# twice154/ofa-for-super-resolution

Hardware: AMD Instinct MI355X
Metric: sr_training_images_per_sec_4x_64to256 (higher is better)
Workload: dtype bf16; 1 GPU; OFA-SR S4 supernet 4x progressive shrinking (elastic kernel {3,5,7}, e=6, d=4, pd=2), LR 64x64 -> HR 256x256, fwd+bwd+Adam, train-mode BN; kernel_transform_mode=1, compat_reference_indexing=True, parallelism=dp1, per_gpu_batch=16, global_batch=16, grad_allreduce_bytes=0, launch=eager

## Files before the change

### ofa-for-super-resolution_amd/csrc/dwconv.hip

```cpp
#include "ofasr_common.h"

#include <type_traits>

namespace ofasr {

constexpr int DW_WAVES = 4;

template <int D>
__device__ __forceinline__ float lane_shift(float v, int lane) {
    if (D == 0) return v;
    const int src = lane + D;
    const float t = __shfl(v, src & 63, 64);
    return (src >= 0 && src < 64) ? t : 0.f;
}

template <int K>
struct Strips {
    static constexpr int PAD = K / 2;
    static __host__ __device__ int count(int W) { return W <= 64 ? 1 : (W + (64 - 2 * PAD) - 1) / (64 - 2 * PAD); }
    static __device__ int col0(int W, int s) { return W <= 64 ? 0 : s * (64 - 2 * PAD) - PAD; }
    static __device__ bool core(int W, int lane) { return W <= 64 ? true : (lane >= PAD && lane < 64 - PAD); }
};

template <typename T, int K, bool FLIP>
__global__ void __launch_bounds__(64 * DW_WAVES) dw_strip_kernel(const T* __restrict__ x, const float* __restrict__ f,
                                                                 T* __restrict__ y, int C, int H, int W,
                                                                 int nstrips, int nchunks, int rows_per_chunk,
                                                                 long long units) {
    constexpr int PAD = K / 2;
    const int lane = lane_id();
    const int wave = __builtin_amdgcn_readfirstlane((int)(threadIdx.x >> 6));
    const long long unit = (long long)blockIdx.x * DW_WAVES + wave;
    if (unit >= units) return;
    const int chunk = (int)(unit % nchunks);
    const long long u2 = unit / nchunks;
    const int strip = (int)(u2 % nstrips);
    const long long plane = u2 / nstrips;
    const int c = (int)(plane % C);

    float taps[K * K];
#pragma unroll
    for (int e = 0; e < K * K; ++e) taps[e] = f[(long long)c * K * K + (FLIP ? (K * K - 1 - e) : e)];

    const int col = Strips<K>::col0(W, strip) + lane;
    const bool in_col = col >= 0 && col < W;
    const bool out_col = in_col && Strips<K>::core(W, lane);
    const int h0 = chunk * rows_per_chunk;
    const int h1 = min(H, h0 + rows_per_chunk);
    const T* xp = x + plane * (long long)H * W + col;
    T* yp = y + plane * (long long)H * W + col;

    float acc[K];
#pragma unroll
    for (int i = 0; i < K; ++i) acc[i] = 0.f;

    const int hstart = h0 - PAD;
    const int niter = (h1 - h0) + 2 * PAD;
    auto load_row = [&](int t) -> float {
        const int hin = hstart + t;
        return (t < niter && hin >= 0 && hin < H && in_col) ? to_float(xp[(long long)hin * W]) : 0.f;
    };
    float xin[K], xnext[K];
#pragma unroll
    for (int u = 0; u < K; ++u) xin[u] = load_row(u);
    for (int base = 0; base < niter; base += K) {
#pragma unroll
        for (int u = 0; u < K; ++u) xnext[u] = load_row(base + K + u);
#pragma unroll
        for (int u = 0; u < K; ++u) {
            const int t = base + u;
            const int hin = hstart + t;
            const float v = xin[u];
            float s[K];
#pragma unroll
            for (int j = 0; j < K; ++j) {
                switch (j - PAD) {
                    case -3: s[j] = lane_shift<-3>(v, lane); break;
                    case -2: s[j] = lane_shift<-2>(v, lane); break;
                    case -1: s[j] = lane_shift<-1>(v, lane); break;
                    case 0: s[j] = v; break;
                    case 1: s[j] = lane_shift<1>(v, lane); break;
                    case 2: s[j] = lane_shift<2>(v, lane); break;
                    default: s[j] = lane_shift<3>(v, lane); break;
                }
            }
#pragma unroll
            for (int i = 0; i < K; ++i) {
                float a = acc[(u - i + K) % K];
#pragma unroll
                for (int j = 0; j < K; ++j) a = fmaf(taps[i * K + j], s[j], a);
                acc[(u - i + K) % K] = a;
            }
            const int hout = hin - PAD;
            if (t < niter && hout >= h0 && hout < h1 && out_col)
                yp[(long long)hout * W] = from_float<T>(acc[(u + 1) % K]);
            acc[(u + 1) % K] = 0.f;
        }
#pragma unroll
        for (int u = 0; u < K; ++u) xin[u] = xnext[u];
    }
}

template <typename T, int K>
__global__ void __launch_bounds__(64 * DW_WAVES) dw_wgrad_kernel(const T* __restrict__ dy, const T* __restrict__ x,
                                                                 float* __restrict__ part_out, int N, int C, int H,
                                                                 int W, int nstrips, int nparts, long long units) {
    constexpr int PAD = K / 2;
    const int lane = lane_id();
    const int wave = __builtin_amdgcn_readfirstlane((int)(threadIdx.x >> 6));
    const long long unit = (long long)blockIdx.x * DW_WAVES + wave;
    if (unit >= units) return;
    const int part = (int)(unit % nparts);
    const int c = (int)(unit / nparts);

    float acc[K * K];
#pragma unroll
    for (int e = 0; e < K * K; ++e) acc[e] = 0.f;

    for (int n = part; n < N; n += nparts) {
        const long long plane = (long long)n * C + c;
        for (int strip = 0; strip < nstrips; ++strip) {
            const int col = Strips<K>::col0(W, strip) + lane;
            const bool in_col = col >= 0 && col < W;
            const bool own = in_col && Strips<K>::core(W, lane);
            const T* dp = dy + plane * (long long)H * W + col;
            const T* xp = x + plane * (long long)H * W + col;
            float xr[K];
#pragma unroll
            for (int m = 0; m < K - 1; ++m) {
                const int r = m - PAD;
                xr[m] = (own && r >= 0 && r < H) ? to_float(xp[(long long)r * W]) : 0.f;
            }
            xr[K - 1] = 0.f;
            auto load_x = [&](int h) -> float {
                const int rnew = h + PAD;
                return (own && h < H && rnew < H) ? to_float(xp[(long long)rnew * W]) : 0.f;
            };
            auto load_g = [&](int h) -> float { return (h < H && in_col) ? to_float(dp[(long long)h * W]) : 0.f; };
            float xb[K], gb[K], xn_[K], gn_[K];
#pragma unroll
            for (int u = 0; u < K; ++u) {
                xb[u] = load_x(u);
                gb[u] = load_g(u);
            }
            for (int base = 0; base < H; base += K) {
#pragma unroll
                for (int u = 0; u < K; ++u) {
                    xn_[u] = load_x(base + K + u);
                    gn_[u] = load_g(base + K + u);
                }
#pragma unroll
                for (int u = 0; u < K; ++u) {
                    xr[(u + K - 1) % K] = xb[u];
                    const float g = gb[u];
                    float gs[K];
#pragma unroll
                    for (int j = 0; j < K; ++j) {
                        switch (PAD - j) {
                            case -3: gs[j] = lane_shift<-3>(g, lane); break;
                            case -2: gs[j] = lane_shift<-2>(g, lane); break;
                            case -1: gs[j] = lane_shift<-1>(g, lane); break;
                            case 0: gs[j] = g; break;
                            case 1: gs[j] = lane_shift<1>(g, lane); break;
                            case 2: gs[j] = lane_shift<2>(g, lane); break;
                            default: gs[j] = lane_shift<3>(g, lane); break;
                        }
                    }
#pragma unroll
                    for (int i = 0; i < K; ++i) {
                        const float xv = xr[(u + i) % K];
#pragma unroll
                        for (int j = 0; j < K; ++j) acc[i * K + j] = fmaf(gs[j], xv, acc[i * K + j]);
                    }
                }
#pragma unroll
                for (int u = 0; u < K; ++u) {
                    xb[u] = xn_[u];
                    gb[u] = gn_[u];
                }
            }
        }
    }
    float* out = part_out + ((long long)part * C + c) * (K * K);
#pragma unroll
    for (int e = 0; e < K * K; ++e) {
        const float s = wave_sum(acc[e]);
        if (lane == 0) out[e] = s;
    }
}

template <typename T, int PXL> struct PxIO;
template <> struct PxIO<float, 4> {
    typedef uint4 raw_t;
    static __device__ __forceinline__ raw_t zero() { return make_uint4(0, 0, 0, 0); }
    static __device__ __forceinline__ void unpack(const raw_t& v, float* o) {
        o[0] = __uint_as_float(v.x); o[1] = __uint_as_float(v.y); o[2] = __uint_as_float(v.z); o[3] = __uint_as_float(v.w);
    }
    static __device__ __forceinline__ raw_t pack(const float* i) {
        return make_uint4(__float_as_uint(i[0]), __float_as_uint(i[1]), __float_as_uint(i[2]), __float_as_uint(i[3]));
    }
};
template <typename T> struct PxIO<T, 8> {
    typedef uint4 raw_t;
    static __device__ __forceinline__ raw_t zero() { return make_uint4(0, 0, 0, 0); }
    static __device__ __forceinline__ void unpack(const raw_t& v, float* o) {
        const uint32_t w[4] = {v.x, v.y, v.z, v.w};
#pragma unroll
        for (int i = 0; i < 4; ++i) {
            T lo, hi;
            lo.v = (uint16_t)(w[i] & 0xffffu);
            hi.v = (uint16_t)(w[i] >> 16);
            o[2 * i] = to_float(lo);
            o[2 * i + 1] = to_float(hi);
        }
    }
    static __device__ __forceinline__ raw_t pack(const float* i) {
        return make_uint4(pack2<T>(i[0], i[1]), pack2<T>(i[2], i[3]), pack2<T>(i[4], i[5]), pack2<T>(i[6], i[7]));
    }
};
template <typename T> struct PxIO<T, 4> {
    typedef uint2 raw_t;
    static __device__ __forceinline__ raw_t zero() { return make_uint2(0, 0); }
    static __device__ __forceinline__ void unpack(const raw_t& v, float* o) {
        const uint32_t w[2] = {v.x, v.y};
#pragma unroll
        for (int i = 0; i < 2; ++i) {
            T lo, hi;
            lo.v = (uint16_t)(w[i] & 0xffffu);
            hi.v = (uint16_t)(w[i] >> 16);
            o[2 * i] = to_float(lo);
            o[2 * i + 1] = to_float(hi);
        }
    }
    static __device__ __forceinline__ raw_t pack(const float* i) { return make_uint2(pack2<T>(i[0], i[1]), pack2<T>(i[2], i[3])); }
};

template <typename T, int K> struct VecPx { static constexpr int N = (K <= 3 && sizeof(T) == 2) ? 8 : 4; };

template <int PXL, int PAD>
__device__ __forceinline__ void build_window(const float* v, float* win, int lane, bool has_left, bool has_right) {
#pragma unroll
    for (int i = 0; i < PAD; ++i) {
        const float l = __shfl(v[PXL - PAD + i], (lane + 63) & 63, 64);
        const float r = __shfl(v[i], (lane + 1) & 63, 64);
        win[i] = has_left ? l : 0.f;
        win[PAD + PXL + i] = has_right ? r : 0.f;
    }
#pragma unroll
    for (int i = 0; i < PXL; ++i) win[PAD + i] = v[i];
}

typedef __attribute__((ext_vector_type(16))) float dwm_f32x16;
typedef __attribute__((ext_vector_type(8))) short dwm_s16x8;
typedef __attribute__((ext_vector_type(8))) __bf16 dwm_bf16x8;
typedef __attribute__((ext_vector_type(8))) _Float16 dwm_f16x8;
template <typename T> struct DwMma;
template <> struct DwMma<bf16_t> {
    static __device__ __forceinline__ dwm_f32x16 run(dwm_s16x8 a, dwm_s16x8 b, dwm_f32x16 c) {
        return __builtin_amdgcn_mfma_f32_32x32x16_bf16(__builtin_bit_cast(dwm_bf16x8, a), __builtin_bit_cast(dwm_bf16x8, b),
                                                       c, 0, 0, 0);
    }
};
template <> struct DwMma<f16_t> {
    static __device__ __forceinline__ dwm_f32x16 run(dwm_s16x8 a, dwm_s16x8 b, dwm_f32x16 c) {
        return __builtin_amdgcn_mfma_f32_32x32x16_f16(__builtin_bit_cast(dwm_f16x8, a), __builtin_bit_cast(dwm_f16x8, b), c,
                                                      0, 0, 0);
    }
};
constexpr int DWM_NPW = 4;
constexpr int DWM_PITCH = 144;
__device__ __forceinline__ void dwm_lds_fence() { asm volatile("s_waitcnt lgkmcnt(0)" ::: "memory"); }

template <typename T, int K, bool FLIP, bool XF, bool STAT, bool BX = false>
__global__ void __launch_bounds__(64 * DW_WAVES) dw_mfma_kernel(const T* __restrict__ x, const float* __restrict__ f,
                                                                T* __restrict__ y, int N, int C, int H, int W,
                                                                int nslabs, InputXf xf, StatOut so, BnFold fold,
                                                                BwdXf bx = BwdXf{}) {
    constexpr int PAD = K / 2;
    constexpr int LROWS = 64 + 2 * PAD;
    __shared__ __attribute__((aligned(16))) char planes[DW_WAVES][LROWS * DWM_PITCH];
    __shared__ __attribute__((aligned(16))) char outs[DW_WAVES][64 * 128];
    __shared__ uint16_t tapt[DW_WAVES][K][96];
    const int lane = lane_id();
    const int wave = __builtin_amdgcn_readfirstlane((int)(threadIdx.x >> 6));
    const long long unit = (long long)blockIdx.x * DW_WAVES + wave;
    const int c = (int)(unit % C);
    const int n0 = (int)(unit / C) * DWM_NPW;
    if (n0 >= N) return;
    char* L = planes[wave];
    const int r = lane & 31, hh = lane >> 5;

    for (int i = lane; i < LROWS * (DWM_PITCH / 16); i += 64) *reinterpret_cast<uint4*>(L + i * 16) = make_uint4(0, 0, 0, 0);
    for (int i = lane; i < K * 96; i += 64) tapt[wave][i / 96][i % 96] = 0;
    dwm_lds_fence();
    for (int e = lane; e < K * K; e += 64)
        tapt[wave][e / K][e % K + 40] = from_float<T>(f[(long long)c * K * K + (FLIP ? (K * K - 1 - e) : e)]).v;
    dwm_lds_fence();
    dwm_s16x8 Bf[K][3];
#pragma unroll
    for (int ky = 0; ky < K; ++ky)
#pragma unroll
        for (int ch = 0; ch < 3; ++ch) {
            const int base = (-8 + 16 * ch) + 8 * hh - r + PAD + 40;
            dwm_s16x8 b;
#pragma unroll
            for (int i = 0; i < 8; ++i) b[i] = (short)tapt[wave][ky][base + i];
            Bf[ky][ch] = b;
        }

    float xsc = 1.f, xmu = 0.f, xb = 0.f;
    if constexpr (XF) {
        if (fold.cp) {
            bn_fold_wave(fold, c, lane, n0 == 0 && lane == 0, xsc, xmu, xb);
        } else {
            xsc = xf.scale[c];
            xmu = xf.mean[c];
            xb = bn_beta(xmu, xsc, xf.shift[c]);
        }
    }

    float bmu = 0.f, bsc = 1.f, bxb = 0.f, bka = 0.f, bkbi = 0.f;
    if constexpr (BX) {
        bmu = bx.mean[c];
        bsc = bx.scale[c];
        bxb = bn_beta(bmu, bsc, bx.shift[c]);
        if (bx.fold_partial) bwdxf_fold(bx, c, bsc, n0 == 0 && lane == 0, bka, bkbi);
        else {
            bka = bx.ka[c];
            bkbi = bx.kbi[c];
        }
    }

    int abase[2][3];
#pragma unroll
    for (int wb = 0; wb < 2; ++wb)
#pragma unroll
        for (int ch = 0; ch < 3; ++ch) {
            const int cidx = 4 * wb - 1 + 2 * ch + hh;
            const int cz = (cidx < 0 || cidx >= (W >> 3)) ? 8 : cidx;
            abase[wb][ch] = r * DWM_PITCH + cz * 16;
        }
    const int cpr = W >> 3;
    const int nchunks = H * cpr;
    char* O = outs[wave];
    uint4 nxt[8];
    uint4 nxt2[BX ? 8 : 1];
    auto load_plane = [&](int pl) {
        const long long plane = (long long)(n0 + pl) * C + c;
        const uint4* src = reinterpret_cast<const uint4*>(x + plane * (long long)H * W);
#pragma unroll
        for (int it = 0; it < 8; ++it) {
            const int idx = lane + 64 * it;
            nxt[it] = src[idx < nchunks ? idx : 0];
        }
        if constexpr (BX) {
            const uint4* src2 = reinterpret_cast<const uint4*>(reinterpret_cast<const T*>(bx.y) + plane * (long long)H * W);
#pragma unroll
            for (int it = 0; it < 8; ++it) {
                const int idx = lane + 64 * it;
                nxt2[it] = src2[idx < nchunks ? idx : 0];
            }
        }
    };
    load_plane(0);
    for (int pl = 0; pl < DWM_NPW && n0 + pl < N; ++pl) {
        const long long plane = (long long)(n0 + pl) * C + c;
#pragma unroll
        for (int it = 0; it < 8; ++it) {
            const int idx = lane + 64 * it;
            if (idx < nchunks) {
                uint4 v = nxt[it];
                if constexpr (XF) v = xf_apply8_core<T>(v, xsc, xmu, xb);
                if constexpr (BX) {
                    v = bx_apply8<T>(v, nxt2[it], bmu, bsc, bxb, bka, bkbi);
                    if (bx.dy_out)
                        reinterpret_cast<uint4*>(reinterpret_cast<T*>(bx.dy_out) + plane * (long long)H * W)[idx] = v;
                }
                const int row = idx / cpr, chunk = idx - row * cpr, lr = row + PAD;
                *reinterpret_cast<uint4*>(L + lr * DWM_PITCH + (chunk << 4)) = v;
            }
        }
        dwm_lds_fence();
        if (pl + 1 < DWM_NPW && n0 + pl + 1 < N) load_plane(pl + 1);
        float st_s = 0.f, st_q = 0.f;
        for (int hb = 0; hb < H / 32; ++hb) {
            const char* Lh = L + hb * (32 * DWM_PITCH);
#pragma unroll
            for (int wb = 0; wb < 2; ++wb) {
                if (32 * wb >= W) break;
                dwm_f32x16 acc;
#pragma unroll
                for (int i = 0; i < 16; ++i) acc[i] = 0.f;
#pragma unroll
                for (int ky = 0; ky < K; ++ky) {
#pragma unroll
                    for (int ch = 0; ch < 3; ++ch) {
                        const dwm_s16x8 a =
                            *reinterpret_cast<const dwm_s16x8*>(Lh + abase[wb][ch] + ky * DWM_PITCH);
                        acc = DwMma<T>::run(Bf[ky][ch], a, acc);
                    }
                }
                const int h = 32 * hb + r;
#pragma unroll
                for (int q = 0; q < 4; ++q) {
                    const uint2 o = make_uint2(pack2<T>(acc[4 * q], acc[4 * q + 1]), pack2<T>(acc[4 * q + 2], acc[4 * q + 3]));
                    const int chunk = 4 * wb + q;
                    *reinterpret_cast<uint2*>(O + h * 128 + ((chunk ^ ((h >> 1) & 7)) << 4) + 8 * hh) = o;
                    if constexpr (STAT) {
                        const uint32_t wv2[2] = {o.x, o.y};
#pragma unroll
                        for (int i = 0; i < 2; ++i) {
                            T lo, hi;
                            lo.v = (uint16_t)(wv2[i] & 0xffffu);
                            hi.v = (uint16_t)(wv2[i] >> 16);
                            const float a0 = to_float(lo), a1 = to_float(hi);
                            st_s += a0 + a1;
                            st_q = fmaf(a0, a0, fmaf(a1, a1, st_q));
                        }
                    }
                }
            }
        }
        dwm_lds_fence();
        uint4* dst = reinterpret_cast<uint4*>(y + plane * (long long)H * W);
#pragma unroll
        for (int it = 0; it < 8; ++it) {
            const int idx = lane + 64 * it;
            if (idx < nchunks) {
                const int row = idx / cpr, chunk = idx - row * cpr;
                dst[idx] = *reinterpret_cast<const uint4*>(O + row * 128 + ((chunk ^ ((row >> 1) & 7)) << 4));
            }
        }
        dwm_lds_fence();
        if constexpr (STAT) {
            const float s = wave_sum(st_s), q = wave_sum(st_q);
            if (lane == 0) {
                so.partial[(long long)c * so.P + (long long)(n0 + pl) * nslabs] = make_float2(s, q);
                for (int sl = 1; sl < nslabs; ++sl)
                    so.partial[(long long)c * so.P + (long long)(n0 + pl) * nslabs + sl] = make_float2(0.f, 0.f);
            }
        }
    }
}

static bool mfma_geom_ok(int64_t H, int64_t W, int K, const void* a, const void* b) {
    const uintptr_t bits = reinterpret_cast<uintptr_t>(a) | reinterpret_cast<uintptr_t>(b);
    return K >= 5 && (W == 32 || W == 64) && H >= 32 && H <= 64 && (H % 32) == 0 && (bits & 15) == 0;
}

struct VecGeom {
    int G, gpw, R, nslabs;
};

template <typename T, int K, bool FLIP, bool XF = false, bool STAT = false, bool BX = false>
__global__ void __launch_bounds__(64 * DW_WAVES) dw_vec_kernel(const T* __restrict__ x, const float* __restrict__ f,
                                                               T* __restrict__ y, int C, int H, int W, VecGeom vg,
                                                               long long nwaves, InputXf xf = InputXf{},
                                                               StatOut so = StatOut{nullptr, 0}, BnFold fold = BnFold{},
                                                               BwdXf bx = BwdXf{}) {
    constexpr int PAD = K / 2;
    constexpr int PXL = VecPx<T, K>::N;
    typedef PxIO<T, PXL> IO;
    typedef typename IO::raw_t raw_t;
    const int lane = lane_id();
    const int wave = __builtin_amdgcn_readfirstlane((int)(threadIdx.x >> 6));
    const long long wunit = (long long)blockIdx.x * DW_WAVES + wave;
    if (wunit >= nwaves) return;
    const int slab = (int)(wunit % vg.nslabs);
    const long long plane = wunit / vg.nslabs;
    const int c = (int)(plane % C);

    float taps[K * K];
#pragma unroll
    for (int e = 0; e < K * K; ++e) taps[e] = f[(long long)c * K * K + (FLIP ? (K * K - 1 - e) : e)];
    float bmu = 0.f, bsc = 1.f, bxb = 0.f, bka = 0.f, bkbi = 0.f;
    if constexpr (BX) {
        bmu = bx.mean[c];
        bsc = bx.scale[c];
        bxb = bn_beta(bmu, bsc, bx.shift[c]);
        if (bx.fold_partial) bwdxf_fold(bx, c, bsc, plane < C && slab == 0 && lane == 0, bka, bkbi);
        else {
            bka = bx.ka[c];
            bkbi = bx.kbi[c];
        }
    }
    float xsc = 1.f, xmu = 0.f, xb = 0.f;
    if constexpr (XF) {
        if (fold.cp) {
            bn_fold_wave(fold, c, lane, plane < C && slab == 0 && lane == 0, xsc, xmu, xb);
        } else {
            xsc = xf.scale[c];
            xmu = xf.mean[c];
            xb = bn_beta(xmu, xsc, xf.shift[c]);
        }
    }

    const int g = lane / vg.G, gl = lane - g * vg.G;
    const bool live = g < vg.gpw;
    const int h0 = min(H, (slab * vg.gpw + g) * vg.R);
    const int h1 = live ? min(H, h0 + vg.R) : h0;
    const int Wq = W / PXL;
    const raw_t* xp = reinterpret_cast<const raw_t*>(x + plane * (long long)H * W) + gl;
    raw_t* yp = reinterpret_cast<raw_t*>(y + plane * (long long)H * W) + gl;
    const bool has_left = gl > 0, has_right = gl < vg.G - 1;

    float acc[K][PXL];
#pragma unroll
    for (int i = 0; i < K; ++i)
#pragma unroll
        for (int p = 0; p < PXL; ++p) acc[i][p] = 0.f;

    float st_s = 0.f, st_q = 0.f;
    const int hstart = h0 - PAD;
    const int niter_max = vg.R + 2 * PAD;
    const int niter = (h1 - h0) + 2 * PAD;
    auto load_row = [&](int t) -> raw_t {
        const int hin = hstart + t;
        return (live && t < niter && hin >= 0 && hin < H) ? xp[(long long)hin * Wq] : IO::zero();
    };
    const raw_t* yp2 = BX ? reinterpret_cast<const raw_t*>(reinterpret_cast<const T*>(bx.y) + plane * (long long)H * W) + gl : nullptr;
    auto load_row2 = [&](int t) -> raw_t {
        const int hin = hstart + t;
        return (BX && live && t < niter && hin >= 0 && hin < H) ? yp2[(long long)hin * Wq] : IO::zero();
    };
    raw_t raw[K];
    raw_t raw2[BX ? K : 1];
#pragma unroll
    for (int u = 0; u < K; ++u) {
        raw[u] = load_row(u);
        if constexpr (BX) raw2[u] = load_row2(u);
    }
    for (int base = 0; base < niter_max; base += K) {
#pragma unroll
        for (int u = 0; u < K; ++u) {
            const int t = base + u;
            const int hin = hstart + t;
            float v[PXL], win[PXL + 2 * PAD + 1];
            IO::unpack(raw[u], v);
            if constexpr (XF) {
                const bool rv = live && t < niter && hin >= 0 && hin < H;
#pragma unroll
                for (int p = 0; p < PXL; ++p) v[p] = rv ? relu6(bn_pre(v[p], xmu, xsc, xb)) : 0.f;
            }
            if constexpr (BX) {
                float yv[PXL];
                IO::unpack(raw2[u], yv);
                const bool rv = live && t < niter && hin >= 0 && hin < H;
#pragma unroll
                for (int p = 0; p < PXL; ++p) {
                    const float dz = relu6_gate(bn_pre(yv[p], bmu, bsc, bxb), v[p]);
                    v[p] = rv ? bn_bwd_dy(yv[p] - bmu, dz, bsc, bka, bkbi) : 0.f;
                }
                raw2[u] = load_row2(t + K);
                if (bx.dy_out && rv && hin >= h0 && hin < h1)
                    (reinterpret_cast<raw_t*>(reinterpret_cast<T*>(bx.dy_out) + plane * (long long)H * W) + gl)[(long long)hin * Wq] = IO::pack(v);
            }
            raw[u] = load_row(t + K);
            build_window<PXL, PAD>(v, win, lane, has_left, has_right);
#pragma unroll
            for (int i = 0; i < K; ++i) {
                if (t - i >= 0 && t - i < vg.R) {
#pragma unroll
                    for (int p = 0; p < PXL; ++p) {
                        float a = acc[(u - i + K) % K][p];
#pragma unroll
                        for (int j = 0; j < K; ++j) a = fmaf(taps[i * K + j], win[p + j], a);
                        acc[(u - i + K) % K][p] = a;
                    }
                }
            }
            const int hout = hin - PAD;
            if (t < niter && hout >= h0 && hout < h1) {
                const raw_t o = IO::pack(acc[(u + 1) % K]);
                yp[(long long)hout * Wq] = o;
                if constexpr (STAT) {
                    float r[PXL];
                    IO::unpack(o, r);
#pragma unroll
                    for (int p = 0; p < PXL; ++p) {
                        st_s += r[p];
                        st_q = fmaf(r[p], r[p], st_q);
                    }
                }
            }
#pragma unroll
            for (int p = 0; p < PXL; ++p) acc[(u + 1) % K][p] = 0.f;
        }
    }
    if constexpr (STAT) {
        const float s = wave_sum(st_s), q = wave_sum(st_q);
        if (lane == 0) so.partial[(long long)c * so.P + (plane / C) * vg.nslabs + slab] = make_float2(s, q);
    }
}

template <typename T, int K, bool XF = false>
__global__ void __launch_bounds__(64 * DW_WAVES) dw_wgrad_vec_kernel(const T* __restrict__ dy, const T* __restrict__ x,
                                                                     float* __restrict__ part_out, int H, int W,
                                                                     VecGeom vg, long long nwaves, int C = 1,
                                                                     InputXf xf = InputXf{}) {
    constexpr int PAD = K / 2;
    constexpr int PXL = 4;
    typedef PxIO<T, PXL> IO;
    typedef typename IO::raw_t raw_t;
    const int lane = lane_id();
    const int wave = __builtin_amdgcn_readfirstlane((int)(threadIdx.x >> 6));
    const long long wunit = (long long)blockIdx.x * DW_WAVES + wave;
    if (wunit >= nwaves) return;
    const int slab = (int)(wunit % vg.nslabs);
    const long long plane = wunit / vg.nslabs;
    const int g = lane / vg.G, gl = lane - g * vg.G;
    const bool live = g < vg.gpw;
    const int h0 = min(H, (slab * vg.gpw + g) * vg.R);
    const int h1 = live ? min(H, h0 + vg.R) : h0;
    const int Wq = W / PXL;
    const raw_t* dp = reinterpret_cast<const raw_t*>(dy + plane * (long long)H * W) + gl;
    const raw_t* xp = reinterpret_cast<const raw_t*>(x + plane * (long long)H * W) + gl;
    const bool has_left = gl > 0, has_right = gl < vg.G - 1;

    float acc[K * K];
#pragma unroll
    for (int e = 0; e < K * K; ++e) acc[e] = 0.f;
    float xr[K][PXL];
    auto load_x = [&](int r) -> raw_t { return xp[(long long)(r < 0 ? 0 : (r < H ? r : H - 1)) * Wq]; };
    auto load_g = [&](int h) -> raw_t { return dp[(long long)(h < H ? h : H - 1) * Wq]; };
    auto x_ok = [&](int r) { return live && r >= 0 && r < H; };
    float xsc = 1.f, xmu = 0.f, xb = 0.f;
    if constexpr (XF) {
        const int c = (int)(plane % C);
        xsc = xf.scale[c];
        xmu = xf.mean[c];
        xb = bn_beta(xmu, xsc, xf.shift[c]);
    }
    auto xform = [&](float* v, int r) {
        const bool rv = x_ok(r);
        if constexpr (XF) {
#pragma unroll
            for (int p = 0; p < PXL; ++p) v[p] = rv ? relu6(bn_pre(v[p], xmu, xsc, xb)) : 0.f;
        } else {
#pragma unroll
            for (int p = 0; p < PXL; ++p) v[p] = rv ? v[p] : 0.f;
        }
    };
#pragma unroll
    for (int m = 0; m < K - 1; ++m) {
        IO::unpack(load_x(h0 - PAD + m), xr[m]);
        xform(xr[m], h0 - PAD + m);
    }
#pragma unroll
    for (int p = 0; p < PXL; ++p) xr[K - 1][p] = 0.f;
    raw_t rawx[K], rawg[K];
#pragma unroll
    for (int u = 0; u < K; ++u) {
        rawx[u] = load_x(h0 + u + PAD);
        rawg[u] = load_g(h0 + u);
    }
    for (int base = 0; base < vg.R; base += K) {
#pragma unroll
        for (int u = 0; u < K; ++u) {
            const int h = h0 + base + u;
            float gv[PXL], gwin[PXL + 2 * PAD + 1];
            IO::unpack(rawx[u], xr[(u + K - 1) % K]);
            xform(xr[(u + K - 1) % K], h + PAD);
            IO::unpack(rawg[u], gv);
            if (h >= h1) {
#pragma unroll
                for (int p = 0; p < PXL; ++p) gv[p] = 0.f;
            }
            rawx[u] = load_x(h + K + PAD);
            rawg[u] = load_g(h + K);
            build_window<PXL, PAD>(gv, gwin, lane, has_left, has_right);
            if (base + u < vg.R) {
#pragma unroll
                for (int i = 0; i < K; ++i)
#pragma unroll
                    for (int j = 0; j < K; ++j) {
                        float a = acc[i * K + j];
#pragma unroll
                        for (int p = 0; p < PXL; ++p) a = fmaf(xr[(u + i) % K][p], gwin[p + K - 1 - j], a);
                        acc[i * K + j] = a;
                    }
            }
        }
    }
    float* out = part_out + wunit * (K * K);
#pragma unroll
    for (int e = 0; e < K * K; ++e) {
        const float s = wave_sum(acc[e]);
        if (lane == 0) out[e] = s;
    }
}

__global__ void __launch_bounds__(256) dw_wgrad_vec_reduce_kernel(const float* __restrict__ part, float* __restrict__ df,
                                                                  int N, int C, int nslabs, int KK) {
    const long long idx = (long long)blockIdx.x * blockDim.x + threadIdx.x;
    if (idx >= (long long)C * KK) return;
    const int c = (int)(idx / KK), e = (int)(idx - (long long)c * KK);
    float s = 0.f;
    for (int n = 0; n < N; ++n)
        for (int q = 0; q < nslabs; ++q) s += part[(((long long)n * C + c) * nslabs + q) * KK + e];
    df[idx] = s;
}

static bool vec_geom(int64_t H, int64_t W, int esize, int PXL, const void* a, const void* b, VecGeom& vg) {
    const uintptr_t bits = reinterpret_cast<uintptr_t>(a) | reinterpret_cast<uintptr_t>(b);
    if (H <= 0 || W <= 0 || W % PXL != 0 || W / PXL > 64 || (bits & 15) != 0) return false;
    (void)esize;
    vg.G = (int)(W / PXL);
    vg.gpw = 64 / vg.G;
    int64_t R = cdiv(H, vg.gpw);
    if (R < 4) R = 4;
    if (R > 32) R = 32;
    vg.R = (int)R;
    vg.nslabs = (int)cdiv(H, (int64_t)vg.gpw * vg.R);
    return true;
}

__global__ void __launch_bounds__(256) dw_wgrad_reduce_kernel(const float* __restrict__ part_out,
                                                              float* __restrict__ df, int nparts, long long CKK) {
    const long long idx = (long long)blockIdx.x * blockDim.x + threadIdx.x;
    if (idx >= CKK) return;
    float s = 0.f;
    for (int p = 0; p < nparts; ++p) s += part_out[(long long)p * CKK + idx];
    df[idx] = s;
}

static int wgrad_parts(int64_t N, int64_t C) {
    int64_t want = cdiv(6144, C > 0 ? C : 1);
    if (want < 1) want = 1;
    if (want > N) want = N;
    return (int)want;
}

template <typename T, bool FLIP, bool XF = false, bool STAT = false, bool BX = false>
static int launch_conv(const char* name, const void* x, const float* f, void* y, int64_t N, int64_t C, int64_t H,
// ... 465 lines not shown
```

Measured before the change: 2832 images/s.

## Software-pipeline LDS fragment loads in depthwise MFMA kernel with a register ring

Restructures the depthwise MFMA conv kernel. The first plane's global load and the tap weight fetch are issued before LDS zeroing and BN fold setup, so their latency overlaps that work. The tile loop is flattened and uses a ring of K prefetched A-fragments, loading the next tile's fragments while the current MFMAs issue, with sched_barriers pinning the order. Index math and bounds checks are replaced by shifts, masks and unconditional clamped loads, and output stores are batched. This trades more registers and fixed schedules, which may cut occupancy, for hidden LDS and global latency.

```diff
diff --git a/ofa-for-super-resolution_amd/csrc/dwconv.hip b/ofa-for-super-resolution_amd/csrc/dwconv.hip
--- a/ofa-for-super-resolution_amd/csrc/dwconv.hip
+++ b/ofa-for-super-resolution_amd/csrc/dwconv.hip
@@ -289,24 +289,34 @@
     if (n0 >= N) return;
     char* L = planes[wave];
     const int r = lane & 31, hh = lane >> 5;
-
+    const int cpr = W >> 3;
+    const int csh = W == 64 ? 3 : 2;
+    const int nchunks = H * cpr;
+    const int nit = nchunks >> 6;
+    const int npl = min(DWM_NPW, N - n0);
+
+    uint4 nxt[8];
+    uint4 nxt2[BX ? 8 : 1];
+    auto load_plane = [&](int pl) {
+        const bool more = pl < npl;
+        const long long plane = (long long)(n0 + (more ? pl : npl - 1)) * C + c;
+        const int keep = more ? -1 : 7;
+        const uint4* src = reinterpret_cast<const uint4*>(x + plane * (long long)H * W);
+#pragma unroll
+        for (int it = 0; it < 8; ++it) nxt[it] = src[(lane + (it < nit ? 64 * it : 0)) & keep];
+        if constexpr (BX) {
+            const uint4* src2 = reinterpret_cast<const uint4*>(reinterpret_cast<const T*>(bx.y) + plane * (long long)H * W);
+#pragma unroll
+            for (int it = 0; it < 8; ++it) nxt2[it] = src2[(lane + (it < nit ? 64 * it : 0)) & keep];
+        }
+    };
+    load_plane(0);
+    static_assert(K * K <= 64, "one tap per lane");
+    const int te = lane < K * K ? lane : 0;
+    const float tapv = f[(long long)c * K * K + (FLIP ? (K * K - 1 - te) : te)];
+    __builtin_amdgcn_sched_barrier(0);
     for (int i = lane; i < LROWS * (DWM_PITCH / 16); i += 64) *reinterpret_cast<uint4*>(L + i * 16) = make_uint4(0, 0, 0, 0);
     for (int i = lane; i < K * 96; i += 64) tapt[wave][i / 96][i % 96] = 0;
-    dwm_lds_fence();
-    for (int e = lane; e < K * K; e += 64)
-        tapt[wave][e / K][e % K + 40] = from_float<T>(f[(long long)c * K * K + (FLIP ? (K * K - 1 - e) : e)]).v;
-    dwm_lds_fence();
-    dwm_s16x8 Bf[K][3];
-#pragma unroll
-    for (int ky = 0; ky < K; ++ky)
-#pragma unroll
-        for (int ch = 0; ch < 3; ++ch) {
-            const int base = (-8 + 16 * ch) + 8 * hh - r + PAD + 40;
-            dwm_s16x8 b;
-#pragma unroll
-            for (int i = 0; i < 8; ++i) b[i] = (short)tapt[wave][ky][base + i];
-            Bf[ky][ch] = b;
-        }
 
     float xsc = 1.f, xmu = 0.f, xb = 0.f;
     if constexpr (XF) {
@@ -331,6 +341,21 @@
         }
     }
 
+    dwm_lds_fence();
+    if (lane < K * K) tapt[wave][lane / K][lane % K + 40] = from_float<T>(tapv).v;
+    dwm_lds_fence();
+    dwm_s16x8 Bf[K][3];
+#pragma unroll
+    for (int ky = 0; ky < K; ++ky)
+#pragma unroll
+        for (int ch = 0; ch < 3; ++ch) {
+            const int base = (-8 + 16 * ch) + 8 * hh - r + PAD + 40;
+            dwm_s16x8 b;
+#pragma unroll
+            for (int i = 0; i < 8; ++i) b[i] = (short)tapt[wave][ky][base + i];
+            Bf[ky][ch] = b;
+        }
+
     int abase[2][3];
 #pragma unroll
     for (int wb = 0; wb < 2; ++wb)
@@ -340,96 +365,98 @@
             const int cz = (cidx < 0 || cidx >= (W >> 3)) ? 8 : cidx;
             abase[wb][ch] = r * DWM_PITCH + cz * 16;
         }
-    const int cpr = W >> 3;
-    const int nchunks = H * cpr;
     char* O = outs[wave];
-    uint4 nxt[8];
-    uint4 nxt2[BX ? 8 : 1];
-    auto load_plane = [&](int pl) {
+    constexpr int NF = 3 * K;
+    constexpr int DWM_D = K;
+    static_assert(NF % DWM_D == 0, "ring slots are static across tiles");
+    const int nwb = W >> 5, ntiles = (H >> 5) * nwb;
+    auto tile_base = [&](int t, int (&p)[3]) {
+        const int hb = nwb == 2 ? t >> 1 : t, wb = nwb == 2 ? (t & 1) : 0;
+#pragma unroll
+        for (int ch = 0; ch < 3; ++ch) p[ch] = hb * (32 * DWM_PITCH) + (wb ? abase[1][ch] : abase[0][ch]);
+    };
+    auto frag = [&](const int (&p)[3], int i) -> dwm_s16x8 {
+        return *reinterpret_cast<const dwm_s16x8*>(L + p[i % 3] + (i / 3) * DWM_PITCH);
+    };
+    for (int pl = 0; pl < npl; ++pl) {
         const long long plane = (long long)(n0 + pl) * C + c;
-        const uint4* src = reinterpret_cast<const uint4*>(x + plane * (long long)H * W);
-#pragma unroll
-        for (int it = 0; it < 8; ++it) {
+        auto build = [&](int it) {
             const int idx = lane + 64 * it;
-            nxt[it] = src[idx < nchunks ? idx : 0];
-        }
-        if constexpr (BX) {
-            const uint4* src2 = reinterpret_cast<const uint4*>(reinterpret_cast<const T*>(bx.y) + plane * (long long)H * W);
-#pragma unroll
-            for (int it = 0; it < 8; ++it) {
-                const int idx = lane + 64 * it;
-                nxt2[it] = src2[idx < nchunks ? idx : 0];
-            }
-        }
-    };
-    load_plane(0);
-    for (int pl = 0; pl < DWM_NPW && n0 + pl < N; ++pl) {
-        const long long plane = (long long)(n0 + pl) * C + c;
-#pragma unroll
-        for (int it = 0; it < 8; ++it) {
-            const int idx = lane + 64 * it;
-            if (idx < nchunks) {
-                uint4 v = nxt[it];
-                if constexpr (XF) v = xf_apply8_core<T>(v, xsc, xmu, xb);
-                if constexpr (BX) {
-                    v = bx_apply8<T>(v, nxt2[it], bmu, bsc, bxb, bka, bkbi);
-                    if (bx.dy_out)
-                        reinterpret_cast<uint4*>(reinterpret_cast<T*>(bx.dy_out) + plane * (long long)H * W)[idx] = v;
-                }
-                const int row = idx / cpr, chunk = idx - row * cpr, lr = row + PAD;
-                *reinterpret_cast<uint4*>(L + lr * DWM_PITCH + (chunk << 4)) = v;
-            }
-        }
+            uint4 v = nxt[it];
+            if constexpr (XF) v = xf_apply8_core<T>(v, xsc, xmu, xb);
+            if constexpr (BX) {
+                v = bx_apply8<T>(v, nxt2[it], bmu, bsc, bxb, bka, bkbi);
+                if (bx.dy_out)
+                    reinterpret_cast<uint4*>(reinterpret_cast<T*>(bx.dy_out) + plane * (long long)H * W)[idx] = v;
+            }
+            const int row = idx >> csh, chunk = idx & (cpr - 1), lr = row + PAD;
+            *reinterpret_cast<uint4*>(L + lr * DWM_PITCH + (chunk << 4)) = v;
+        };
+        build(0), build(1);
+        if (nit > 2) build(2), build(3);
+        if (nit > 4) build(4), build(5), build(6), build(7);
         dwm_lds_fence();
-        if (pl + 1 < DWM_NPW && n0 + pl + 1 < N) load_plane(pl + 1);
+        load_plane(pl + 1);
         float st_s = 0.f, st_q = 0.f;
-        for (int hb = 0; hb < H / 32; ++hb) {
-            const char* Lh = L + hb * (32 * DWM_PITCH);
-#pragma unroll
-            for (int wb = 0; wb < 2; ++wb) {
-                if (32 * wb >= W) break;
-                dwm_f32x16 acc;
-#pragma unroll
-                for (int i = 0; i < 16; ++i) acc[i] = 0.f;
-#pragma unroll
-                for (int ky = 0; ky < K; ++ky) {
-#pragma unroll
-                    for (int ch = 0; ch < 3; ++ch) {
-                        const dwm_s16x8 a =
-                            *reinterpret_cast<const dwm_s16x8*>(Lh + abase[wb][ch] + ky * DWM_PITCH);
-                        acc = DwMma<T>::run(Bf[ky][ch], a, acc);
+        int pa[3];
+        tile_base(0, pa);
+        dwm_s16x8 ring[DWM_D];
+#pragma unroll
+        for (int d = 0; d < DWM_D; ++d) ring[d] = frag(pa, d);
+        for (int t = 0; t < ntiles; ++t) {
+            int pn[3];
+            tile_base(t, pa);
+            tile_base(t + 1 < ntiles ? t + 1 : t, pn);
+            dwm_f32x16 acc;
+#pragma unroll
+            for (int i = 0; i < 16; ++i) acc[i] = 0.f;
+            __builtin_amdgcn_sched_barrier(0);
+#pragma unroll
+            for (int i = 0; i < NF; ++i) {
+                acc = DwMma<T>::run(Bf[i / 3][i % 3], ring[i % DWM_D], acc);
+                __builtin_amdgcn_sched_barrier(0);
+                ring[i % DWM_D] = i + DWM_D < NF ? frag(pa, i + DWM_D) : frag(pn, i + DWM_D - NF);
+                __builtin_amdgcn_sched_barrier(0);
+            }
+            const int hb = nwb == 2 ? t >> 1 : t, wb = nwb == 2 ? (t & 1) : 0;
+            const int h = 32 * hb + r;
+#pragma unroll
+            for (int q = 0; q < 4; ++q) {
+                const uint2 o = make_uint2(pack2<T>(acc[4 * q], acc[4 * q + 1]), pack2<T>(acc[4 * q + 2], acc[4 * q + 3]));
+                const int chunk = 4 * wb + q;
+                *reinterpret_cast<uint2*>(O + h * 128 + ((chunk ^ ((h >> 1) & 7)) << 4) + 8 * hh) = o;
+                if constexpr (STAT) {
+                    const uint32_t wv2[2] = {o.x, o.y};
+#pragma unroll
+                    for (int i = 0; i < 2; ++i) {
+                        T lo, hi;
+                        lo.v = (uint16_t)(wv2[i] & 0xffffu);
+                        hi.v = (uint16_t)(wv2[i] >> 16);
+                        const float a0 = to_float(lo), a1 = to_float(hi);
+                        st_s += a0 + a1;
+                        st_q = fmaf(a0, a0, fmaf(a1, a1, st_q));
                     }
                 }
-                const int h = 32 * hb + r;
-#pragma unroll
-                for (int q = 0; q < 4; ++q) {
-                    const uint2 o = make_uint2(pack2<T>(acc[4 * q], acc[4 * q + 1]), pack2<T>(acc[4 * q + 2], acc[4 * q + 3]));
-                    const int chunk = 4 * wb + q;
-                    *reinterpret_cast<uint2*>(O + h * 128 + ((chunk ^ ((h >> 1) & 7)) << 4) + 8 * hh) = o;
-                    if constexpr (STAT) {
-                        const uint32_t wv2[2] = {o.x, o.y};
-#pragma unroll
-                        for (int i = 0; i < 2; ++i) {
-                            T lo, hi;
-                            lo.v = (uint16_t)(wv2[i] & 0xffffu);
-                            hi.v = (uint16_t)(wv2[i] >> 16);
-                            const float a0 = to_float(lo), a1 = to_float(hi);
-                            st_s += a0 + a1;
-                            st_q = fmaf(a0, a0, fmaf(a1, a1, st_q));
-                        }
-                    }
-                }
+                __builtin_amdgcn_sched_barrier(0);
             }
         }
         dwm_lds_fence();
         uint4* dst = reinterpret_cast<uint4*>(y + plane * (long long)H * W);
-#pragma unroll
-        for (int it = 0; it < 8; ++it) {
+        auto oread = [&](int it) -> uint4 {
             const int idx = lane + 64 * it;
-            if (idx < nchunks) {
-                const int row = idx / cpr, chunk = idx - row * cpr;
-                dst[idx] = *reinterpret_cast<const uint4*>(O + row * 128 + ((chunk ^ ((row >> 1) & 7)) << 4));
-            }
+            const int row = idx >> csh, chunk = idx & (cpr - 1);
+            return *reinterpret_cast<const uint4*>(O + row * 128 + ((chunk ^ ((row >> 1) & 7)) << 4));
+        };
+        {
+            const uint4 o0 = oread(0), o1 = oread(1), o2 = oread(nit > 2 ? 2 : 0), o3 = oread(nit > 2 ? 3 : 1);
+            __builtin_amdgcn_sched_barrier(0);
+            dst[lane] = o0, dst[lane + 64] = o1;
+            if (nit > 2) dst[lane + 128] = o2, dst[lane + 192] = o3;
+        }
+        if (nit > 4) {
+            const uint4 o4 = oread(4), o5 = oread(5), o6 = oread(6), o7 = oread(7);
+            __builtin_amdgcn_sched_barrier(0);
+            dst[lane + 256] = o4, dst[lane + 320] = o5, dst[lane + 384] = o6, dst[lane + 448] = o7;
         }
         dwm_lds_fence();
         if constexpr (STAT) {
```

Result: no change. 2841 images/s, median of 3 (+0.3%).
